# 2361098148/LocoManipulationRL

Hardware: AMD Instinct MI355X
Metric: env-steps/sec (whole node), horizontal-locomotion 4096 envs (higher is better)
Workload: dtype f32

## Files before the change

locomanipulationrl_amd/csrc/lm_dynamics.h:

```cpp
#pragma once
#include "lm_samplers.h"

#if defined(LM_STAMPS) && LM_STAMPS != 2
#define LM_STAMP(k) do { __builtin_amdgcn_sched_barrier(0); unsigned long long t_; \
    asm volatile("s_memtime %0\n\ts_waitcnt lgkmcnt(0)" : "=s"(t_) :: "memory"); __builtin_amdgcn_sched_barrier(0); \
    if (threadIdx.x == 0) { lm_stamp_lds[k] += t_ - lm_stamp_lds[15]; lm_stamp_lds[15] = t_; } } while (0)
#else
#define LM_STAMP(k) do { } while (0)
#endif

#define HUB_FLOATS 10
#define ENVS_PER_WAVE 16
#define PUB_LIMB_STRIDE 123
#define LIMB_STRIDE 124
#define T_J0 0
#define T_P1 14
#define T_P2 40
#define T_I0 66
#define T_Q1 76
#define T_Q2 96
#define T_TIP 116
#define T_FOOT 119
#define T_FLAG 122
#define LM_ITAB_FLOATS (HUB_FLOATS + 4 * LIMB_STRIDE)
// ... 150 lines not shown
  D.H[3] = Hdd.x + 2.0f * g1 * Hdp.x + gg; D.H[4] = -g1 * (Hdp.x + Hdp.y) - gg; D.H[5] = Hdd.y + 2.0f * g1 * Hdp.y + gg;
  const bool on2 = tl[T_FLAG] != 0.f;
  const V3 off = v3(tl[T_FOOT], tl[T_FOOT + 1], tl[T_FOOT + 2]);
  const SV s2 = lo(K.s23), s3 = hi(K.s23), sp1 = lo(K.sp12), sp2_ = hi(K.sp12);
  D.j31 = sel(on2, (-g1) * sp2_, fma6(g1, sp1, s2));
  D.j32 = sel(on2, fma6(g1, sp2_, s3), (-g1) * sp1);
  D.x = sel(on2, hi(K.o32), lo(K.o32)) + mul(M3{sel(on2, hi(K.R32.c0), lo(K.R32.c0)), sel(on2, hi(K.R32.c1), lo(K.R32.c1)), sel(on2, hi(K.R32.c2), lo(K.R32.c2))}, off);
}

struct PgsData { f2 W0t, nrWt; float X0[4][3]; f2 X12[4][3]; };

struct R4 { f2 p, q; };
struct S6 { f2 a, b, c; };
LM_DEV S6 operator*(float s, S6 x) { const f2 t = sp2(s); S6 r; r.a = t * x.a; r.b = t * x.b; r.c = t * x.c; return r; }
LM_DEV S6 fma6(float s, S6 x, S6 y) { const f2 t = sp2(s); S6 r; r.a = fma_(t, x.a, y.a); r.b = fma_(t, x.b, y.b); r.c = fma_(t, x.c, y.c); return r; }
template <int I> LM_DEV float comp(const S6& x) { return I == 0 ? x.a.x : I == 1 ? x.a.y : I == 2 ? x.b.x : I == 3 ? x.b.y : I == 4 ? x.c.x : x.c.y; }
template <int J> LM_DEV f2 pairc(const S6& x) { return J == 0 ? x.a : J == 1 ? x.b : x.c; }

struct Chol6 { float L[6][6]; float d[6]; };
LM_DEV void chol6(const float A[6][6], Chol6& C) {
#pragma unroll
  for (int j = 0; j < 6; j++) {
    float s = A[j][j];
#pragma unroll
    for (int k = 0; k < j; k++) s = fmaf(-C.L[j][k], C.L[j][k], s);
    const float inv = __builtin_amdgcn_rsqf(s);
    C.d[j] = inv;
#pragma unroll
    for (int i = j + 1; i < 6; i++) {
      float t = A[j][i];
#pragma unroll
      for (int k = 0; k < j; k++) t = fmaf(-C.L[i][k], C.L[j][k], t);
      C.L[i][j] = t * inv;
    }
  }
}
LM_DEV void chol6_solve4(const Chol6& C, R4 x[6]) {
#pragma unroll
  for (int i = 0; i < 6; i++) {
    f2 p = x[i].p, q = x[i].q;
#pragma unroll
    for (int k = 0; k < i; k++) { const f2 l = sp2(-C.L[i][k]); p = fma_(l, x[k].p, p); q = fma_(l, x[k].q, q); }
    const f2 d = sp2(C.d[i]); x[i].p = p * d; x[i].q = q * d;
  }
#pragma unroll
  for (int i = 5; i >= 0; i--) {
    f2 p = x[i].p, q = x[i].q;
#pragma unroll
    for (int k = i + 1; k < 6; k++) { const f2 l = sp2(-C.L[k][i]); p = fma_(l, x[k].p, p); q = fma_(l, x[k].q, q); }
    const f2 d = sp2(C.d[i]); x[i].p = p * d; x[i].q = q * d;
  }
}

template <int K>
LM_DEV void pgs_cross_blocks(int limb, const R4 T[6], const R4 X[6], const float Wf[6], float X0[3], f2 X12[3]) {
  float a00 = 0.f; f2 a0t = sp2(0.f), c0 = sp2(0.f), c1 = sp2(0.f), c2 = sp2(0.f);
#pragma unroll
  for (int i = 0; i < 6; i++) {
    const float k0 = quad_bcast<K>(X[i].p.y); const f2 k12 = mk2(quad_bcast<K>(X[i].q.x), quad_bcast<K>(X[i].q.y));
    const float t0 = T[i].p.y; const f2 t12 = T[i].q;
    a00 = fmaf(t0, k0, a00); a0t = fma_(sp2(t0), k12, a0t);
    c0 = fma_(t12, sp2(k0), c0); c1 = fma_(t12, sp2(k12.x), c1); c2 = fma_(t12, sp2(k12.y), c2);
  }
  const bool own = (limb == K);
  X0[0] = own ? Wf[0] : a00; X0[1] = own ? Wf[1] : a0t.x; X0[2] = own ? Wf[2] : a0t.y;
  X12[0] = mk2(own ? Wf[1] : c0.x, own ? Wf[2] : c0.y);
  X12[1] = mk2(own ? Wf[3] : c1.x, own ? Wf[4] : c1.y);
  X12[2] = mk2(own ? Wf[4] : c2.x, own ? Wf[5] : c2.y);
}

template <int K>
LM_DEV void pgs_turn(float m, const PgsData& G, float& lam0, f2& lam12, float& c0, f2& c12) {
  const float d0 = __builtin_amdgcn_fmed3f(c0, -lam0, __builtin_inff());
  lam0 = fmaf(m, d0, lam0);
  const f2 u12 = fma_(fma_(G.W0t, sp2(d0), c12), G.nrWt, lam12);
  const float sc = fminf(1.0f, lam0 * __builtin_amdgcn_rsqf(fmaf(u12.x, u12.x, u12.y * u12.y)));
  const f2 d12 = fma_(u12, sp2(sc), -lam12);
  lam12 = fma_(sp2(m), d12, lam12);
  const float b0 = quad_bcast<K>(d0), b1 = quad_bcast<K>(d12.x), b2 = quad_bcast<K>(d12.y);
  c0 = fmaf(G.X0[K][2], b2, fmaf(G.X0[K][1], b1, fmaf(G.X0[K][0], b0, c0)));
  c12 = fma_(G.X12[K][2], sp2(b2), fma_(G.X12[K][1], sp2(b1), fma_(G.X12[K][0], sp2(b0), c12)));
}

struct PgsState { PgsData G; float lam0; f2 lam12; float c0; f2 c12; float m0, m1, m2, m3; };
LM_DEV void pgs_setup(PgsState& S, int limb, float mu, float bn, const float vf[3], const float Wl[6], const R4 T[6], const R4 X[6]) {
  PgsData& G = S.G; float Wf[6];
  {
    f2 a0 = sp2(0.f), a1 = sp2(0.f), a2 = sp2(0.f); float b0 = 0.f;
#pragma unroll
    for (int i = 0; i < 6; i++) {
      b0 = fmaf(T[i].p.y, X[i].p.y, b0);
      a0 = fma_(sp2(T[i].p.y), X[i].q, a0); a1 = fma_(sp2(T[i].q.x), X[i].q, a1); a2 = fma_(sp2(T[i].q.y), X[i].q, a2);
    }
    Wf[0] = Wl[0] + b0; Wf[1] = Wl[1] + a0.x; Wf[2] = Wl[2] + a0.y;
    Wf[3] = Wl[3] + a1.x; Wf[4] = Wl[4] + a1.y; Wf[5] = Wl[5] + a2.y;
  }
  const float imu = mu > 0.f ? 1.0f / mu : 0.f;
  const float nrW0 = -1.0f / Wf[0]; G.W0t = mk2(Wf[1], Wf[2]); G.nrWt = mk2(-imu / Wf[3], -imu / Wf[5]);
  pgs_cross_blocks<0>(limb, T, X, Wf, G.X0[0], G.X12[0]); pgs_cross_blocks<1>(limb, T, X, Wf, G.X0[1], G.X12[1]);
  pgs_cross_blocks<2>(limb, T, X, Wf, G.X0[2], G.X12[2]); pgs_cross_blocks<3>(limb, T, X, Wf, G.X0[3], G.X12[3]);
#pragma unroll
  for (int k = 0; k < 4; k++) { G.X0[k][0] *= nrW0; G.X0[k][1] *= mu * nrW0; G.X0[k][2] *= mu * nrW0; G.X12[k][1] = sp2(mu) * G.X12[k][1]; G.X12[k][2] = sp2(mu) * G.X12[k][2]; }
  S.lam0 = 0.f; S.lam12 = sp2(0.f);
  S.c0 = (vf[0] + bn) * nrW0; S.c12 = mk2(vf[1], vf[2]);
  S.m0 = limb == 0 ? 1.f : 0.f; S.m1 = limb == 1 ? 1.f : 0.f; S.m2 = limb == 2 ? 1.f : 0.f; S.m3 = limb == 3 ? 1.f : 0.f;
}
LM_DEV void pgs_sweeps(PgsState& S, int it0, int it1) {
  for (int it = it0; it < it1; it += 2) {
    pgs_turn<0>(S.m0, S.G, S.lam0, S.lam12, S.c0, S.c12);
    pgs_turn<1>(S.m1, S.G, S.lam0, S.lam12, S.c0, S.c12);
    pgs_turn<2>(S.m2, S.G, S.lam0, S.lam12, S.c0, S.c12);
    pgs_turn<3>(S.m3, S.G, S.lam0, S.lam12, S.c0, S.c12);
    if (it + 1 < it1) {
      pgs_turn<3>(S.m3, S.G, S.lam0, S.lam12, S.c0, S.c12);
      pgs_turn<2>(S.m2, S.G, S.lam0, S.lam12, S.c0, S.c12);
      pgs_turn<1>(S.m1, S.G, S.lam0, S.lam12, S.c0, S.c12);
      pgs_turn<0>(S.m0, S.G, S.lam0, S.lam12, S.c0, S.c12);
    }
  }
}
LM_DEV void pgs_finish(const PgsState& S, float mu, const R4 X[6], float lam[3], float w[6]) {
  const f2 l12 = sp2(mu) * S.lam12;
  lam[0] = S.lam0; lam[1] = l12.x; lam[2] = l12.y;
#pragma unroll
  for (int i = 0; i < 6; i++) { const f2 t = l12 * X[i].q; w[i] = quad_sum(fmaf(S.lam0, X[i].p.y, t.x + t.y)); }
}

struct FreeBody { V3 p; Q4 q; SV u; };

LM_DEV void integrate_free(FreeBody& F, const M3& R, float dt) {
  V3 ww = mul(R, F.u.w);
  float wn = sqrtf(dot(ww, ww)), th = wn * dt;
  Q4 dq;
  if (th < 1e-8f) { dq.w = 1.f; dq.x = 0.5f * dt * ww.x; dq.y = 0.5f * dt * ww.y; dq.z = 0.5f * dt * ww.z; }
  else { float sh, ch; lm_sincos(0.5f * th, &sh, &ch); float s = sh / wn; dq.w = ch; dq.x = s * ww.x; dq.y = s * ww.y; dq.z = s * ww.z; }
  Q4 qn = qmul(dq, F.q);
  float rn = rsqrtf(qn.w * qn.w + qn.x * qn.x + qn.y * qn.y + qn.z * qn.z);
  F.q.w = qn.w * rn; F.q.x = qn.x * rn; F.q.y = qn.y * rn; F.q.z = qn.z * rn;
  M3 Rn = quat_to_mat(F.q.w, F.q.x, F.q.y, F.q.z);
  F.p = fma3(dt, mul(Rn, F.u.v), F.p);
}

#ifdef LM_WAVES2
#define STASH_SLOTS 18
#define LM_STEP_ATTR __attribute__((amdgpu_waves_per_eu(2, 2)))
#elif defined(LM_HELPER_WAVE)
#if LM_HELPER_WAVE >= 2
#define STASH_SLOTS 34
#define TASK_SLOT 29
#else
#define STASH_SLOTS 29
#endif
#define HAND_IN 22
#define HAND_OUT 26
#define LM_STEP_ATTR
#else
#define STASH_SLOTS 22
#define LM_STEP_ATTR
#endif
struct Stash {
  float4* base; int lane;
  LM_DEV void put(int slot, float a, float b, float c, float d) const { base[slot * 64 + lane] = make_float4(a, b, c, d); }
  LM_DEV float4 get(int slot) const { return base[slot * 64 + lane]; }
};
#ifdef LM_HELPER_WAVE
LM_DEV void hw_barrier() {
  __builtin_amdgcn_sched_barrier(0);
  asm volatile("" ::: "memory");
  __builtin_amdgcn_s_waitcnt(0xc07f);
  __builtin_amdgcn_s_barrier();
  asm volatile("" ::: "memory");
  __builtin_amdgcn_sched_barrier(0);
}
#endif
LM_DEV void stash_sv3(const Stash& S, int slot, SV a, SV b, SV c, float e0 = 0.f, float e1 = 0.f) {
  S.put(slot + 0, a.w.x, a.w.y, a.w.z, a.v.x); S.put(slot + 1, a.v.y, a.v.z, b.w.x, b.w.y);
  S.put(slot + 2, b.w.z, b.v.x, b.v.y, b.v.z); S.put(slot + 3, c.w.x, c.w.y, c.w.z, c.v.x); S.put(slot + 4, c.v.y, c.v.z, e0, e1);
}
LM_DEV void unstash_sv3(const Stash& S, int slot, SV& a, SV& b, SV& c) {
  float4 t0 = S.get(slot), t1 = S.get(slot + 1), t2 = S.get(slot + 2), t3 = S.get(slot + 3), t4 = S.get(slot + 4);
  a = sv(v3(t0.x, t0.y, t0.z), v3(t0.w, t1.x, t1.y)); b = sv(v3(t1.z, t1.w, t2.x), v3(t2.y, t2.z, t2.w)); c = sv(v3(t3.x, t3.y, t3.z), v3(t3.w, t4.x, t4.y));
}

#if defined(LM_PASS0_STASH) || defined(LM_WAVES2)
#define LM_PASS0_REG 0
#else
#define LM_PASS0_REG 1
#endif
struct PassTerms {
  S6 Fq0, Fq1, Fq2;
  float Ha[6], hq[3];
  float Jq0[3]; f2 j12[3];
  R4 PB[6];
  SI Isc;
};
LM_DEV S6 s6(SV a) { S6 r; r.a = mk2(a.w.x, a.w.y); r.b = mk2(a.w.z, a.v.x); r.c = mk2(a.v.y, a.v.z); return r; }
#define LM_PASS_ROWS(I, b, r0, r1, r2) { \
  I.PB[0].p = mk2(b.w.x, r0.w.x); I.PB[1].p = mk2(b.w.y, r0.w.y); I.PB[2].p = mk2(b.w.z, r0.w.z); \
  I.PB[3].p = mk2(b.v.x, r0.v.x); I.PB[4].p = mk2(b.v.y, r0.v.y); I.PB[5].p = mk2(b.v.z, r0.v.z); \
  I.PB[0].q = mk2(r1.w.x, r2.w.x); I.PB[1].q = mk2(r1.w.y, r2.w.y); I.PB[2].q = mk2(r1.w.z, r2.w.z); \
  I.PB[3].q = mk2(r1.v.x, r2.v.x); I.PB[4].q = mk2(r1.v.y, r2.v.y); I.PB[5].q = mk2(r1.v.z, r2.v.z); }
LM_DEV void pin(float& x) { asm("" : "+v"(x)); }
// ... 38 lines not shown
  St.put(4, I.Fq2.c.x, I.Fq2.c.y, 0.f, 0.f);
  St.put(5, I.Ha[0], I.Ha[1], I.Ha[2], I.Ha[3]); St.put(6, I.Ha[4], I.Ha[5], 0.f, 0.f);
  St.put(16, I.Isc.m, I.Isc.h.x, I.Isc.h.y, I.Isc.h.z); St.put(17, I.Isc.xx, I.Isc.yy, I.Isc.zz, I.Isc.xy); St.put(18, I.Isc.xz, I.Isc.yz, 0.f, 0.f);
}
#endif
template <int MODE> LM_DEV void unstash_terms(const Stash& St, PassTerms& I) {
  asm volatile("" ::: "memory");
  float isc_xz = 0.f, isc_yz = 0.f;
  {
    const float4 t0 = St.get(0), t1 = St.get(1), t2 = St.get(2), t3 = St.get(3), t4 = St.get(4);
    isc_xz = t4.z; isc_yz = t4.w;
    I.Fq0.a = mk2(t0.x, t0.y); I.Fq0.b = mk2(t0.z, t0.w); I.Fq0.c = mk2(t1.x, t1.y);
    I.Fq1.a = mk2(t1.z, t1.w); I.Fq1.b = mk2(t2.x, t2.y); I.Fq1.c = mk2(t2.z, t2.w);
    I.Fq2.a = mk2(t3.x, t3.y); I.Fq2.b = mk2(t3.z, t3.w); I.Fq2.c = mk2(t4.x, t4.y);
  }
  const float4 h5 = St.get(5), h6 = St.get(6), h7 = St.get(7), h8 = St.get(8), h9 = St.get(9);
  I.Ha[0] = h5.x; I.Ha[1] = h5.y; I.Ha[2] = h5.z; I.Ha[3] = h5.w; I.Ha[4] = h6.x; I.Ha[5] = h6.y;
  I.hq[0] = h6.z; I.hq[1] = h6.w; I.hq[2] = h7.x;
  I.Jq0[0] = h7.y; I.Jq0[1] = h7.z; I.Jq0[2] = h7.w;
  I.j12[0] = mk2(h8.x, h8.y); I.j12[1] = mk2(h8.z, h8.w); I.j12[2] = mk2(h9.x, h9.y);
  {
    const float4 g0 = St.get(10), g1 = St.get(11), g2 = St.get(12), g3 = St.get(13), g4 = St.get(14), g5 = St.get(15);
    I.PB[0].p = mk2(g0.x, g0.y); I.PB[1].p = mk2(g0.z, g0.w); I.PB[2].p = mk2(g1.x, g1.y); I.PB[3].p = mk2(g1.z, g1.w); I.PB[4].p = mk2(g2.x, g2.y); I.PB[5].p = mk2(g2.z, g2.w);
    I.PB[0].q = mk2(g3.x, g3.y); I.PB[1].q = mk2(g3.z, g3.w); I.PB[2].q = mk2(g4.x, g4.y); I.PB[3].q = mk2(g4.z, g4.w); I.PB[4].q = mk2(g5.x, g5.y); I.PB[5].q = mk2(g5.z, g5.w);
  }
  if (MODE == 0) {
#ifdef LM_WAVES2
    const float4 g16 = St.get(16), g17 = St.get(17), g18 = make_float4(isc_xz, isc_yz, 0.f, 0.f);
#else
    const float4 g16 = St.get(16), g17 = St.get(17), g18 = St.get(18); (void)isc_xz; (void)isc_yz;
#endif
    I.Isc.m = g16.x; I.Isc.h = v3(g16.y, g16.z, g16.w); I.Isc.xx = g17.x; I.Isc.yy = g17.y; I.Isc.zz = g17.z; I.Isc.xy = g17.w; I.Isc.xz = g18.x; I.Isc.yz = g18.y;
  }
}

template <class T> struct PlateInvT { V3T<T> ii, c; T im; };
LM_DEV PlateInvT<float> plate_inv(const lm_params* __restrict__ P, float m, float s) {
  PlateInvT<float> Q; Q.ii = v3(1.0f / (s * P->plate_inertia[0]), 1.0f / (s * P->plate_inertia[1]), 1.0f / (s * P->plate_inertia[2]));
  Q.c = v3(P->plate_com[0], P->plate_com[1], P->plate_com[2]); Q.im = 1.0f / m; return Q;
}
template <class T> LM_DEV void plate_inv_apply(const PlateInvT<T>& Q, V3T<T> n, V3T<T> f, V3T<T>& al, V3T<T>& a) {
  const V3T<T> nc = n - cross(Q.c, f);
  al = v3t<T>(nc.x * Q.ii.x, nc.y * Q.ii.y, nc.z * Q.ii.z);
  a = fma3(Q.im, f, cross(Q.c, al));
}
LM_DEV SI plate_inertia_env(const lm_params* __restrict__ P, float m, float s) {
  const V3 c = v3(P->plate_com[0], P->plate_com[1], P->plate_com[2]); const float cc = dot(c, c);
  SI I; I.m = m; I.h = m * c;
  I.xx = fmaf(m, cc - c.x * c.x, s * P->plate_inertia[0]); I.yy = fmaf(m, cc - c.y * c.y, s * P->plate_inertia[1]); I.zz = fmaf(m, cc - c.z * c.z, s * P->plate_inertia[2]);
  I.xy = -m * c.x * c.y; I.xz = -m * c.x * c.z; I.yz = -m * c.y * c.z;
  return I;
}

template <int MODE, int VAR, int DR, int CF, int HW = 0>
LM_DEV void substep_pass(const lm_params* __restrict__ P, int limb, const FreeBody& F, const PassTerms& I, float dt, float kd, const float cjv[3],
                         const bool sat[3], const float tsat[3], const float tgt[3], const float qd[3], float bn, float mu_dr,
                         bool mp_on, float m_plate, float s_plate, float qdn[3], SV& un, float lamc[3], const Stash* Hd = nullptr) {
  const S6 Fq0 = I.Fq0, Fq1 = I.Fq1, Fq2 = I.Fq2;
  float Ha[6] = {I.Ha[0], I.Ha[1], I.Ha[2], I.Ha[3], I.Ha[4], I.Ha[5]}, r[3];
  const float hq[3] = {I.hq[0], I.hq[1], I.hq[2]};
  R4 PBh[6];
  const float Jq_[3][3] = {{I.Jq0[0], I.Jq0[1], I.Jq0[2]}, {I.j12[0].x, I.j12[1].x, I.j12[2].x}, {I.j12[0].y, I.j12[1].y, I.j12[2].y}};
  const f2 j12_[3] = {I.j12[0], I.j12[1], I.j12[2]};
  float Jqh[3][3]; f2 j12h[3]; float bnh = bn;
  const float (*Jq)[3] = HW == 2 ? Jqh : Jq_;
  const f2* j12 = HW == 2 ? j12h : j12_;
  const R4* PB = HW ? PBh : I.PB;
  const int di[3] = {0, 3, 5};
#pragma unroll
  for (int a = 0; a < 3; a++) {
    const float cj = cjv[a];
    {
#pragma clang fp contract(off)
      Ha[di[a]] = fmaf(dt, sat[a] ? cj : kd + cj, Ha[di[a]]);
      const float rr = sat[a] ? tsat[a] : kd * (tgt[a] - qd[a]);
      const float damp = cj * qd[a];
      r[a] = HW ? rr - damp : (rr - damp) - hq[a];
    }
  }
  float Hi[6]; inv3sym(Ha, Hi);
  const S6 K0 = fma6(Hi[0], Fq0, fma6(Hi[1], Fq1, Hi[2] * Fq2));
  const S6 K1 = fma6(Hi[1], Fq0, fma6(Hi[3], Fq1, Hi[4] * Fq2));
  const S6 K2 = fma6(Hi[2], Fq0, fma6(Hi[4], Fq1, Hi[5] * Fq2));
  float qdd[3], qdf[3], v0f[6], vf[3];
  R4 T[6], X[6];
  if (MODE == 0) {
    float A0[6][6]; si_to_66(I.Isc, A0);
    float A[6][6];
#define LM_AROW(I) { \
      const f2 k0 = sp2(comp<I>(K0)), k1 = sp2(comp<I>(K1)), k2 = sp2(comp<I>(K2)); \
      _Pragma("unroll") for (int jp = (I) / 2; jp < 3; jp++) { \
        const f2 f0 = jp == 0 ? Fq0.a : jp == 1 ? Fq0.b : Fq0.c, f1 = jp == 0 ? Fq1.a : jp == 1 ? Fq1.b : Fq1.c, f2_ = jp == 0 ? Fq2.a : jp == 1 ? Fq2.b : Fq2.c; \
        const f2 v = fma_(-k2, f2_, fma_(-k1, f1, fma_(-k0, f0, mk2(A0[I][2 * jp], A0[I][2 * jp + 1])))); \
        if (2 * jp >= (I)) A[I][2 * jp] = quad_sum(v.x); \
        A[I][2 * jp + 1] = quad_sum(v.y); } }
    LM_AROW(0) LM_AROW(1) LM_AROW(2) LM_AROW(3) LM_AROW(4) LM_AROW(5)
#undef LM_AROW
#ifdef LM_HELPER_WAVE
    if (HW) {
      hw_barrier();
      const float4 b0 = Hd->get(HAND_OUT), b1 = Hd->get(HAND_OUT + 1), b2 = Hd->get(HAND_OUT + 2);
      const float fcs[6] = {b0.x, b0.y, b0.z, b0.w, b1.x, b1.y}, hqh[3] = {b1.z, b1.w, b2.x};
      if (HW == 2) {
        const float4 t7 = Hd->get(7), t8 = Hd->get(8), t9 = Hd->get(9);
        const float4 g0 = Hd->get(10), g1 = Hd->get(11), g2 = Hd->get(12), g3 = Hd->get(13), g4 = Hd->get(14), g5 = Hd->get(15);
        j12h[0] = mk2(t8.x, t8.y); j12h[1] = mk2(t8.z, t8.w); j12h[2] = mk2(t9.x, t9.y); bnh = t9.z;
        Jqh[0][0] = t7.y; Jqh[0][1] = t7.z; Jqh[0][2] = t7.w;
#pragma unroll
        for (int c = 0; c < 3; c++) { Jqh[1][c] = j12h[c].x; Jqh[2][c] = j12h[c].y; }
        PBh[0].p = mk2(fcs[0], g0.y); PBh[1].p = mk2(fcs[1], g0.w); PBh[2].p = mk2(fcs[2], g1.y);
        PBh[3].p = mk2(fcs[3], g1.w); PBh[4].p = mk2(fcs[4], g2.y); PBh[5].p = mk2(fcs[5], g2.w);
        PBh[0].q = mk2(g3.x, g3.y); PBh[1].q = mk2(g3.z, g3.w); PBh[2].q = mk2(g4.x, g4.y);
        PBh[3].q = mk2(g4.z, g4.w); PBh[4].q = mk2(g5.x, g5.y); PBh[5].q = mk2(g5.z, g5.w);
      } else {
#pragma unroll
      for (int i = 0; i < 6; i++) { PBh[i].p = mk2(fcs[i], I.PB[i].p.y); PBh[i].q = I.PB[i].q; }
      }
#pragma unroll
      for (int a = 0; a < 3; a++) {
#pragma clang fp contract(off)
        r[a] = r[a] - hqh[a];
      }
    }
#endif
    Chol6 Ch; chol6(A, Ch);
    const f2 cp[3] = {mk2(r[0], -Jq[0][0]), mk2(r[1], -Jq[0][1]), mk2(r[2], -Jq[0][2])};
#define LM_PROW(I) { \
      const f2 k0 = sp2(comp<I>(K0)), k1 = sp2(comp<I>(K1)), k2 = sp2(comp<I>(K2)); \
      T[I].p = fma_(cp[2], k2, fma_(cp[1], k1, fma_(cp[0], k0, PB[I].p))); \
      T[I].q = fma_(-j12[2], k2, fma_(-j12[1], k1, fma_(-j12[0], k0, PB[I].q))); \
      X[I].p = mk2(-quad_sum(T[I].p.x), T[I].p.y); X[I].q = T[I].q; }
    LM_PROW(0) LM_PROW(1) LM_PROW(2) LM_PROW(3) LM_PROW(4) LM_PROW(5)
#undef LM_PROW
    chol6_solve4(Ch, X);
    float t0 = r[0], t1 = r[1], t2 = r[2];
#define LM_TROW(I) { const float a = X[I].p.x; t0 = fmaf(-comp<I>(Fq0), a, t0); t1 = fmaf(-comp<I>(Fq1), a, t1); t2 = fmaf(-comp<I>(Fq2), a, t2); }
    LM_TROW(0) LM_TROW(1) LM_TROW(2) LM_TROW(3) LM_TROW(4) LM_TROW(5)
#undef LM_TROW
    qdd[0] = Hi[0] * t0 + Hi[1] * t1 + Hi[2] * t2; qdd[1] = Hi[1] * t0 + Hi[3] * t1 + Hi[4] * t2; qdd[2] = Hi[2] * t0 + Hi[4] * t1 + Hi[5] * t2;
    const float u6[6] = {F.u.w.x, F.u.w.y, F.u.w.z, F.u.v.x, F.u.v.y, F.u.v.z};
#pragma unroll
    for (int i = 0; i < 6; i++) v0f[i] = fmaf(dt, X[i].p.x, u6[i]);
  } else {
    qdd[0] = Hi[0] * r[0] + Hi[1] * r[1] + Hi[2] * r[2]; qdd[1] = Hi[1] * r[0] + Hi[3] * r[1] + Hi[4] * r[2]; qdd[2] = Hi[2] * r[0] + Hi[4] * r[1] + Hi[5] * r[2];
#pragma unroll
    for (int i = 0; i < 6; i++) { v0f[i] = PB[i].p.x; T[i] = PB[i]; }
    if (mp_on) {
      const PlateInvT<float> Q1 = plate_inv(P, m_plate, s_plate);
      PlateInvT<f2> Q; Q.ii = bc(Q1.ii); Q.c = bc(Q1.c); Q.im = sp2(Q1.im);
      V3P al, ac;
      plate_inv_apply<f2>(Q, v3(T[0].p, T[1].p, T[2].p), v3(T[3].p, T[4].p, T[5].p), al, ac);
      X[0].p = al.x; X[1].p = al.y; X[2].p = al.z; X[3].p = ac.x; X[4].p = ac.y; X[5].p = ac.z;
      plate_inv_apply<f2>(Q, v3(T[0].q, T[1].q, T[2].q), v3(T[3].q, T[4].q, T[5].q), al, ac);
      X[0].q = al.x; X[1].q = al.y; X[2].q = al.z; X[3].q = ac.x; X[4].q = ac.y; X[5].q = ac.z;
    } else {
#pragma unroll
    for (int i = 0; i < 6; i++) {
      f2 bp = sp2(0.f), bq = sp2(0.f);
#pragma unroll
      for (int j = 0; j < 6; j++) { const f2 ph = sp2(P->plate_phi[6 * i + j]); bp = fma_(ph, T[j].p, bp); bq = fma_(ph, T[j].q, bq); }
      X[i].p = bp; X[i].q = bq;
    }
    }
  }
#pragma unroll
  for (int a = 0; a < 3; a++) qdf[a] = fmaf(dt, qdd[a], qd[a]);
  float Wl[6];
  float JH[3][3];
#pragma unroll
  for (int rr = 0; rr < 3; rr++) {
    JH[rr][0] = Jq[rr][0] * Hi[0] + Jq[rr][1] * Hi[1] + Jq[rr][2] * Hi[2];
    JH[rr][1] = Jq[rr][0] * Hi[1] + Jq[rr][1] * Hi[3] + Jq[rr][2] * Hi[4];
    JH[rr][2] = Jq[rr][0] * Hi[2] + Jq[rr][1] * Hi[4] + Jq[rr][2] * Hi[5];
  }
  Wl[0] = JH[0][0] * Jq[0][0] + JH[0][1] * Jq[0][1] + JH[0][2] * Jq[0][2];
  Wl[1] = JH[0][0] * Jq[1][0] + JH[0][1] * Jq[1][1] + JH[0][2] * Jq[1][2];
  Wl[2] = JH[0][0] * Jq[2][0] + JH[0][1] * Jq[2][1] + JH[0][2] * Jq[2][2];
  Wl[3] = JH[1][0] * Jq[1][0] + JH[1][1] * Jq[1][1] + JH[1][2] * Jq[1][2];
  Wl[4] = JH[1][0] * Jq[2][0] + JH[1][1] * Jq[2][1] + JH[1][2] * Jq[2][2];
  Wl[5] = JH[2][0] * Jq[2][0] + JH[2][1] * Jq[2][1] + JH[2][2] * Jq[2][2];
  {
    float a = 0.f; f2 b = sp2(0.f);
#pragma unroll
    for (int i = 0; i < 6; i++) { a = fmaf(PB[i].p.y, v0f[i], a); b = fma_(PB[i].q, sp2(v0f[i]), b); }
    vf[0] = a + (Jq[0][0] * qdf[0] + Jq[0][1] * qdf[1] + Jq[0][2] * qdf[2]);
    vf[1] = b.x + (Jq[1][0] * qdf[0] + Jq[1][1] * qdf[1] + Jq[1][2] * qdf[2]);
    vf[2] = b.y + (Jq[2][0] * qdf[0] + Jq[2][1] * qdf[1] + Jq[2][2] * qdf[2]);
  }
  float lam[3], w[6];
  LM_STAMP(3);
  PgsState S; pgs_setup(S, limb, DR ? mu_dr : P->mu, HW == 2 ? bnh : bn, vf, Wl, T, X);
  pgs_sweeps(S, 0, P->pgs_iters);
  pgs_finish(S, DR ? mu_dr : P->mu, X, lam, w);
  if (CF) { lamc[0] = lam[0]; lamc[1] = lam[1]; lamc[2] = lam[2]; }
  un = sv(v3(v0f[0] + w[0], v0f[1] + w[1], v0f[2] + w[2]), v3(v0f[3] + w[3], v0f[4] + w[4], v0f[5] + w[5]));
#pragma unroll
  for (int a = 0; a < 3; a++) qdn[a] = qdf[a] + JH[0][a] * lam[0] + JH[1][a] * lam[1] + JH[2][a] * lam[2];
  if (MODE == 0) {
#define LM_WROW(I) { qdn[0] = fmaf(-comp<I>(K0), w[I], qdn[0]); qdn[1] = fmaf(-comp<I>(K1), w[I], qdn[1]); qdn[2] = fmaf(-comp<I>(K2), w[I], qdn[2]); }
    LM_WROW(0) LM_WROW(1) LM_WROW(2) LM_WROW(3) LM_WROW(4) LM_WROW(5)
#undef LM_WROW
  }
  LM_STAMP(4);
}

#ifdef LM_HELPER_WAVE
LM_DEV void helper_wave(const lm_params* __restrict__ P, const float* sTab, float4* sStash, int lane, int nsub) {
  const int limb = lane & 3;
  const float* th = sTab; const float* tl = sTab + HUB_FLOATS + limb * LIMB_STRIDE;
  Stash St; St.base = sStash; St.lane = lane;
  const float gravity = P->gravity;
  for (int s = 0; s < nsub; s++) {
    hw_barrier();
    const float4 h0 = St.get(HAND_IN), h1 = St.get(HAND_IN + 1), h2 = St.get(HAND_IN + 2), h3 = St.get(HAND_IN + 3);
    const float q[3] = {h0.x, h0.y, h0.z}, qd[3] = {h0.w, h1.x, h1.y};
    const SV v0 = sv(v3(h1.z, h1.w, h2.x), v3(h2.y, h2.z, h2.w));
    const SV avp0 = sv(v3(0, 0, 0), gravity * v3(h3.x, h3.y, h3.z));
    LimbKin K; limb_kinematics(tl, q, qd, K);
    LimbDyn D; limb_dynamics<0, 2>(tl, K, qd, v0, avp0, D);
    {
      const float m0 = (limb == 0) ? 1.f : 0.f;
      SI I0 = hub_inertia(th);
      I0.m *= m0; I0.h = m0 * I0.h; I0.xx *= m0; I0.yy *= m0; I0.zz *= m0; I0.xy *= m0; I0.xz *= m0; I0.yz *= m0;
      D.fcs = D.fcs + I0 * avp0 + fcross(v0, I0 * v0);
    }
    St.put(HAND_OUT, D.fcs.w.x, D.fcs.w.y, D.fcs.w.z, D.fcs.v.x); St.put(HAND_OUT + 1, D.fcs.v.y, D.fcs.v.z, D.hq[0], D.hq[1]); St.put(HAND_OUT + 2, D.hq[2], 0.f, 0.f, 0.f);
    hw_barrier();
  }
}
#if LM_HELPER_WAVE >= 2
LM_DEV void helper_wave_terms(const lm_params* __restrict__ P, const float* sTab, float4* sStash, int lane, int nsub) {
  const int limb = lane & 3;
  const float* tl = sTab + HUB_FLOATS + limb * LIMB_STRIDE;
  Stash St; St.base = sStash; St.lane = lane;
  const float dt = P->dt, baumgarte = P->baumgarte, max_depen_vel = P->max_depen_vel;
  for (int s = 0; s < nsub; s++) {
    hw_barrier();
    const float4 h0 = St.get(HAND_IN), h1 = St.get(HAND_IN + 1), h2 = St.get(HAND_IN + 2), h3 = St.get(HAND_IN + 3);
    const float q[3] = {h0.x, h0.y, h0.z}, qd[3] = {h0.w, h1.x, h1.y};
    const SV v0 = sv(v3(h1.z, h1.w, h2.x), v3(h2.y, h2.z, h2.w));
    const SV avp0 = sv(v3(0, 0, 0), v3(0, 0, 0));
    LimbKin K; limb_kinematics(tl, q, qd, K);
    LimbDyn D; limb_dynamics<0, 1>(tl, K, qd, v0, avp0, D);
    V3 C0, C1, C2; float phi;
    C0 = v3(h3.x, h3.y, h3.z);
    C1 = rsqrtf(fmaxf(1.0f - C0.x * C0.x, 1.0e-12f)) * v3(1.0f - C0.x * C0.x, -C0.x * C0.y, -C0.x * C0.z);
    C2 = cross(C0, C1);
    phi = h3.w + dot(C0, D.x) - P->tip_radius;
    D.x = fma3(-P->tip_radius, C0, D.x);
    const float bn = (phi >= 0.f) ? phi / dt : fmaxf(baumgarte * phi / dt, -max_depen_vel);
    V3 e0 = K.s1.v + cross(K.s1.w, D.x);
    V3 e1 = D.j31.v + cross(D.j31.w, D.x);
    V3 e2 = D.j32.v + cross(D.j32.w, D.x);
    St.put(7, 0.f, dot(C0, e0), dot(C0, e1), dot(C0, e2));
    St.put(8, dot(C1, e0), dot(C2, e0), dot(C1, e1), dot(C2, e1)); St.put(9, dot(C1, e2), dot(C2, e2), bn, 0.f);
    const V3 n0 = cross(D.x, C0), n1 = cross(D.x, C1), n2 = cross(D.x, C2);
    St.put(10, 0.f, n0.x, 0.f, n0.y); St.put(11, 0.f, n0.z, 0.f, C0.x); St.put(12, 0.f, C0.y, 0.f, C0.z);
    St.put(13, n1.x, n2.x, n1.y, n2.y); St.put(14, n1.z, n2.z, C1.x, C2.x); St.put(15, C1.y, C2.y, C1.z, C2.z);
    hw_barrier();
  }
}
#endif
#endif

template <int MODE, int VAR, int DR, int CF = 0, int REG0 = 1, int HW = 0>
LM_DEV void substep(const lm_params* __restrict__ P, const float* th, const float* tl, int limb, const Stash& St,
                    FreeBody& F, const M3& Rfix, V3 pfix, float q[3], float qd[3], const float tgt[3], float tau_acc[3], const DrPhys& X, float* cf = nullptr) {
  const float dt = P->dt, kd = DR ? X.kd : P->kd;
  const float cjv[3] = {VAR ? (DR ? X.cj[0] : P->joint_damping) : 0.f, VAR ? (DR ? X.cj[1] : P->joint_damping) : 0.f, VAR ? (DR ? X.cj[2] : P->joint_damping) : 0.f};
  const float tmax[3] = {DR ? X.tmax[0] : P->tau_max, DR ? X.tmax[1] : P->tau_max, DR ? X.tmax[2] : P->tau_max};
  const float mu_dr = DR ? X.mu : 0.f;
  const bool mp_on = DR && MODE == 1 && X.mp_on;
  const float m_plate = mp_on ? X.m_plate : 0.f, s_plate = mp_on ? X.s_plate : 0.f;
  M3 Rf = quat_to_mat(F.q.w, F.q.x, F.q.y, F.q.z);
#ifdef LM_HELPER_WAVE
  static_assert(!HW || (MODE == 0 && !DR && LM_PASS0_REG && REG0), "the helper wavefront serves the un-randomised locomotion sub-step with its first pass on registers");
  if (HW) {
    St.put(HAND_IN, q[0], q[1], q[2], qd[0]); St.put(HAND_IN + 1, qd[1], qd[2], F.u.w.x, F.u.w.y); St.put(HAND_IN + 2, F.u.w.z, F.u.v.x, F.u.v.y, F.u.v.z);
    St.put(HAND_IN + 3, Rf.c0.z, Rf.c1.z, Rf.c2.z, HW == 2 ? F.p.z : 0.f);
    hw_barrier();
  }
#endif
  constexpr bool REG0_ = LM_PASS0_REG ? REG0 != 0 : false;
  const float baumgarte = REG0_ ? P->baumgarte : 0.f, max_depen_vel = REG0_ ? P->max_depen_vel : 0.f;
  float bn; PassTerms I;
  {
    M3 Rb; V3 pb; SV v0;
    if (MODE == 0) { Rb = Rf; pb = F.p; v0 = F.u; } else { Rb = Rfix; pb = pfix; v0 = sv(v3(0, 0, 0), v3(0, 0, 0)); }
    SV avp0 = sv(v3(0, 0, 0), DR ? mulT(Rb, -X.g) : P->gravity * row2(Rb));
    LimbKin K; limb_kinematics(tl, q, qd, K);
    LimbDyn D;
    if (DR && X.mb_on) limb_dynamics<1>(tl, K, qd, v0, avp0, D, X.m_s, X.m_41, X.m_32);
    else if (HW) limb_dynamics<0, 1>(tl, K, qd, v0, avp0, D);
    else limb_dynamics(tl, K, qd, v0, avp0, D);
    LM_STAMP(1);
    if (MODE == 0) {
      const float m0 = (limb == 0) ? 1.f : 0.f;
      SI I0 = hub_inertia(th);
      if (DR && X.mb_on) {
        const V3 c = (1.0f / I0.m) * I0.h; const float dm = X.m_hub - I0.m, cc = dot(c, c);
        I0.xx = fmaf(dm, cc - c.x * c.x, I0.xx); I0.yy = fmaf(dm, cc - c.y * c.y, I0.yy); I0.zz = fmaf(dm, cc - c.z * c.z, I0.zz);
        I0.xy = fmaf(dm, -(c.x * c.y), I0.xy); I0.xz = fmaf(dm, -(c.x * c.z), I0.xz); I0.yz = fmaf(dm, -(c.y * c.z), I0.yz);
        I0.h = (X.m_hub / I0.m) * I0.h; I0.m = X.m_hub;
      }
      const V3 com0 = (1.0f / I0.m) * I0.h;
      I0.m *= m0; I0.h = m0 * I0.h; I0.xx *= m0; I0.yy *= m0; I0.zz *= m0; I0.xy *= m0; I0.xz *= m0; I0.yz *= m0;
      D.Isc = D.Isc + I0;
      if (!HW) D.fcs = D.fcs + I0 * avp0 + fcross(v0, I0 * v0);
      if (DR) { V3 fh = m0 * mulT(Rb, X.f); D.fcs = D.fcs - sv(cross(com0, fh), fh); }
    }
#ifdef LM_HELPER_WAVE
    if (HW == 2) {
// ... 192 lines not shown
```

locomanipulationrl_amd/csrc/lm_engine_h3.hip:

```cpp
#ifndef LM_HELPER_WAVE
#define LM_HELPER_WAVE 2
#endif
#ifndef LM_H3_OUT_HELPER
#define LM_H3_OUT_HELPER 1
#endif
#ifndef LM_H3_TAIL_STATE
#define LM_H3_TAIL_STATE 1
#endif
#undef LM_STAMPS
#undef LM_COUNT_PASS2
#undef LM_WAVES2
#undef LM_PASS0_STASH
#include "lm_step.h"

__global__ void __launch_bounds__(192) k_step_h3(StepArgs A) {
  LM_STEP_SMEM(64)
  if (threadIdx.x >= 64) {
    const int nsub = (A.nsub < 0) ? P->substeps : A.nsub;
    if (kind != 0 || env0 >= A.N) return;
    if (threadIdx.x >= 128) {
      helper_wave_terms(P, sTab, sStash, threadIdx.x - 128, nsub);
      if (LM_H3_TAIL_STATE) hw_barrier();
      if (LM_H3_OUT_HELPER) helper_write_outputs<64>(P, A.W, A.N, env0, threadIdx.x - 128, sObs, sSt);
    } else {
      helper_wave(P, sTab, sStash, threadIdx.x - 64, nsub);
      if (LM_H3_TAIL_STATE) helper_task_state(A, P, sStash, threadIdx.x - 64);
    }
    return;
  }
  if (kind == 0) step_body<0, 0, 0, 0, 0, 1, 2, LM_H3_OUT_HELPER, 0, LM_H3_TAIL_STATE>(A, P, sTab, sObs, sSt, sStash); else step_body<1, 0, 0>(A, P, sTab, sObs, sSt, sStash);
}
extern "C" __attribute__((visibility("hidden"))) void lm_internal_launch_step_h3(const StepArgs* A, int nblocks, hipStream_t s) {
  hipLaunchKernelGGL(k_step_h3, dim3(nblocks), dim3(192), 0, s, *A);
}
```

Baseline: 149.9 million.

## Offload PGS cross-limb coupling blocks to helper wavefronts in the h3 kernel

The main wavefront now does the 6x6 Cholesky factorisation first and writes it, together with its K rows, into the LDS stash. The two helper wavefronts each rebuild T and X, do the Cholesky solve and compute the raw cross-limb coupling blocks for two of the four limbs. The main wave then fetches these blocks after a barrier and only applies the per-limb selection and scaling, which takes the per-limb cross-block FMA chains off its critical path. In exchange the stash grows from 34 to 49 slots, there are extra helper barriers every substep, and the solve is repeated on the helper waves. The feature is enabled by default in the h3 engine.

Result: faster. 152.9 million, median of 6 (+2.0%).

```diff
diff --git a/locomanipulationrl_amd/csrc/lm_dynamics.h b/locomanipulationrl_amd/csrc/lm_dynamics.h
--- a/locomanipulationrl_amd/csrc/lm_dynamics.h
+++ b/locomanipulationrl_amd/csrc/lm_dynamics.h
@@ -226,8 +226,9 @@
   }
 }
 
+struct XRaw { float a00; f2 a0t, c0, c1, c2; };
 template <int K>
-LM_DEV void pgs_cross_blocks(int limb, const R4 T[6], const R4 X[6], const float Wf[6], float X0[3], f2 X12[3]) {
+LM_DEV void pgs_cross_raw(const R4 T[6], const R4 X[6], XRaw& R) {
   float a00 = 0.f; f2 a0t = sp2(0.f), c0 = sp2(0.f), c1 = sp2(0.f), c2 = sp2(0.f);
 #pragma unroll
   for (int i = 0; i < 6; i++) {
@@ -236,11 +237,19 @@
     a00 = fmaf(t0, k0, a00); a0t = fma_(sp2(t0), k12, a0t);
     c0 = fma_(t12, sp2(k0), c0); c1 = fma_(t12, sp2(k12.x), c1); c2 = fma_(t12, sp2(k12.y), c2);
   }
+  R.a00 = a00; R.a0t = a0t; R.c0 = c0; R.c1 = c1; R.c2 = c2;
+}
+template <int K>
+LM_DEV void pgs_cross_select(int limb, const XRaw& R, const float Wf[6], float X0[3], f2 X12[3]) {
   const bool own = (limb == K);
-  X0[0] = own ? Wf[0] : a00; X0[1] = own ? Wf[1] : a0t.x; X0[2] = own ? Wf[2] : a0t.y;
-  X12[0] = mk2(own ? Wf[1] : c0.x, own ? Wf[2] : c0.y);
-  X12[1] = mk2(own ? Wf[3] : c1.x, own ? Wf[4] : c1.y);
-  X12[2] = mk2(own ? Wf[4] : c2.x, own ? Wf[5] : c2.y);
+  X0[0] = own ? Wf[0] : R.a00; X0[1] = own ? Wf[1] : R.a0t.x; X0[2] = own ? Wf[2] : R.a0t.y;
+  X12[0] = mk2(own ? Wf[1] : R.c0.x, own ? Wf[2] : R.c0.y);
+  X12[1] = mk2(own ? Wf[3] : R.c1.x, own ? Wf[4] : R.c1.y);
+  X12[2] = mk2(own ? Wf[4] : R.c2.x, own ? Wf[5] : R.c2.y);
+}
+template <int K>
+LM_DEV void pgs_cross_blocks(int limb, const R4 T[6], const R4 X[6], const float Wf[6], float X0[3], f2 X12[3]) {
+  XRaw R; pgs_cross_raw<K>(T, X, R); pgs_cross_select<K>(limb, R, Wf, X0, X12);
 }
 
 template <int K>
@@ -257,7 +266,17 @@
 }
 
 struct PgsState { PgsData G; float lam0; f2 lam12; float c0; f2 c12; float m0, m1, m2, m3; };
-LM_DEV void pgs_setup(PgsState& S, int limb, float mu, float bn, const float vf[3], const float Wl[6], const R4 T[6], const R4 X[6]) {
+#ifndef LM_H3_XBLOCKS
+#define LM_H3_XBLOCKS 0
+#endif
+struct Stash;
+#if defined(LM_HELPER_WAVE) && LM_HELPER_WAVE >= 2
+LM_DEV void xblocks_fetch(const Stash* Hd, XRaw& R0, XRaw& R1, XRaw& R2, XRaw& R3);
+#endif
+LM_DEV void pin_here(float& x) { asm volatile("" : "+v"(x)); }
+LM_DEV void pin_here(f2& x) { asm volatile("" : "+v"(x)); }
+template <int XB = 0>
+LM_DEV void pgs_setup(PgsState& S, int limb, float mu, float bn, const float vf[3], const float Wl[6], const R4 T[6], const R4 X[6], const Stash* Hd = nullptr) {
   PgsData& G = S.G; float Wf[6];
   {
     f2 a0 = sp2(0.f), a1 = sp2(0.f), a2 = sp2(0.f); float b0 = 0.f;
@@ -270,13 +289,25 @@
     Wf[3] = Wl[3] + a1.x; Wf[4] = Wl[4] + a1.y; Wf[5] = Wl[5] + a2.y;
   }
   const float imu = mu > 0.f ? 1.0f / mu : 0.f;
-  const float nrW0 = -1.0f / Wf[0]; G.W0t = mk2(Wf[1], Wf[2]); G.nrWt = mk2(-imu / Wf[3], -imu / Wf[5]);
+  float nrW0 = -1.0f / Wf[0]; G.W0t = mk2(Wf[1], Wf[2]); G.nrWt = mk2(-imu / Wf[3], -imu / Wf[5]);
+#if defined(LM_HELPER_WAVE) && LM_HELPER_WAVE >= 2
+  if (XB) {
+    S.c0 = (vf[0] + bn) * nrW0; S.c12 = mk2(vf[1], vf[2]);
+    pin_here(Wf[0]); pin_here(Wf[1]); pin_here(Wf[2]); pin_here(Wf[3]); pin_here(Wf[4]); pin_here(Wf[5]);
+    pin_here(nrW0); pin_here(G.nrWt); pin_here(S.c0); pin_here(S.c12);
+    XRaw R0, R1, R2, R3; xblocks_fetch(Hd, R0, R1, R2, R3);
+    pgs_cross_select<0>(limb, R0, Wf, G.X0[0], G.X12[0]); pgs_cross_select<1>(limb, R1, Wf, G.X0[1], G.X12[1]);
+    pgs_cross_select<2>(limb, R2, Wf, G.X0[2], G.X12[2]); pgs_cross_select<3>(limb, R3, Wf, G.X0[3], G.X12[3]);
+  } else
+#endif
+  {
   pgs_cross_blocks<0>(limb, T, X, Wf, G.X0[0], G.X12[0]); pgs_cross_blocks<1>(limb, T, X, Wf, G.X0[1], G.X12[1]);
   pgs_cross_blocks<2>(limb, T, X, Wf, G.X0[2], G.X12[2]); pgs_cross_blocks<3>(limb, T, X, Wf, G.X0[3], G.X12[3]);
+  }
 #pragma unroll
   for (int k = 0; k < 4; k++) { G.X0[k][0] *= nrW0; G.X0[k][1] *= mu * nrW0; G.X0[k][2] *= mu * nrW0; G.X12[k][1] = sp2(mu) * G.X12[k][1]; G.X12[k][2] = sp2(mu) * G.X12[k][2]; }
   S.lam0 = 0.f; S.lam12 = sp2(0.f);
-  S.c0 = (vf[0] + bn) * nrW0; S.c12 = mk2(vf[1], vf[2]);
+  if (!XB) { S.c0 = (vf[0] + bn) * nrW0; S.c12 = mk2(vf[1], vf[2]); }
   S.m0 = limb == 0 ? 1.f : 0.f; S.m1 = limb == 1 ? 1.f : 0.f; S.m2 = limb == 2 ? 1.f : 0.f; S.m3 = limb == 3 ? 1.f : 0.f;
 }
 LM_DEV void pgs_sweeps(PgsState& S, int it0, int it1) {
@@ -320,8 +351,15 @@
 #define LM_STEP_ATTR __attribute__((amdgpu_waves_per_eu(2, 2)))
 #elif defined(LM_HELPER_WAVE)
 #if LM_HELPER_WAVE >= 2
+#define TASK_SLOT 29
+#if LM_H3_XBLOCKS
+#define STASH_SLOTS 49
+#define XB_IN_A TASK_SLOT
+#define XB_IN_B 34
+#define XB_OUT 39
+#else
 #define STASH_SLOTS 34
-#define TASK_SLOT 29
+#endif
 #else
 #define STASH_SLOTS 29
 #endif
@@ -466,6 +504,11 @@
   return I;
 }
 
+#define LM_PROW(I, BIAS) { \
+      const f2 k0 = sp2(comp<I>(K0)), k1 = sp2(comp<I>(K1)), k2 = sp2(comp<I>(K2)); \
+      T[I].p = fma_(cp[2], k2, fma_(cp[1], k1, fma_(cp[0], k0, PB[I].p))); \
+      T[I].q = fma_(-j12[2], k2, fma_(-j12[1], k1, fma_(-j12[0], k0, PB[I].q))); \
+      X[I].p = mk2(BIAS, T[I].p.y); X[I].q = T[I].q; }
 template <int MODE, int VAR, int DR, int CF, int HW = 0>
 LM_DEV void substep_pass(const lm_params* __restrict__ P, int limb, const FreeBody& F, const PassTerms& I, float dt, float kd, const float cjv[3],
                          const bool sat[3], const float tsat[3], const float tgt[3], const float qd[3], float bn, float mu_dr,
@@ -510,8 +553,18 @@
         A[I][2 * jp + 1] = quad_sum(v.y); } }
     LM_AROW(0) LM_AROW(1) LM_AROW(2) LM_AROW(3) LM_AROW(4) LM_AROW(5)
 #undef LM_AROW
+    Chol6 Ch;
 #ifdef LM_HELPER_WAVE
     if (HW) {
+#if LM_HELPER_WAVE >= 2 && LM_H3_XBLOCKS
+      if (HW == 2) {
+        chol6(A, Ch);
+        put2(*Hd, XB_IN_A, K0.a, K0.b); put2(*Hd, XB_IN_A + 1, K0.c, K1.a); put2(*Hd, XB_IN_A + 2, K1.b, K1.c); put2(*Hd, XB_IN_A + 3, K2.a, K2.b);
+        Hd->put(XB_IN_A + 4, K2.c.x, K2.c.y, Ch.d[0], Ch.d[1]); Hd->put(XB_IN_B, Ch.d[2], Ch.d[3], Ch.d[4], Ch.d[5]);
+        Hd->put(XB_IN_B + 1, Ch.L[1][0], Ch.L[2][0], Ch.L[2][1], Ch.L[3][0]); Hd->put(XB_IN_B + 2, Ch.L[3][1], Ch.L[3][2], Ch.L[4][0], Ch.L[4][1]);
+        Hd->put(XB_IN_B + 3, Ch.L[4][2], Ch.L[4][3], Ch.L[5][0], Ch.L[5][1]); Hd->put(XB_IN_B + 4, Ch.L[5][2], Ch.L[5][3], Ch.L[5][4], 0.f);
+      }
+#endif
       hw_barrier();
       const float4 b0 = Hd->get(HAND_OUT), b1 = Hd->get(HAND_OUT + 1), b2 = Hd->get(HAND_OUT + 2);
       const float fcs[6] = {b0.x, b0.y, b0.z, b0.w, b1.x, b1.y}, hqh[3] = {b1.z, b1.w, b2.x};
@@ -537,15 +590,10 @@
       }
     }
 #endif
-    Chol6 Ch; chol6(A, Ch);
+    if (!(HW == 2 && LM_H3_XBLOCKS)) chol6(A, Ch);
     const f2 cp[3] = {mk2(r[0], -Jq[0][0]), mk2(r[1], -Jq[0][1]), mk2(r[2], -Jq[0][2])};
-#define LM_PROW(I) { \
-      const f2 k0 = sp2(comp<I>(K0)), k1 = sp2(comp<I>(K1)), k2 = sp2(comp<I>(K2)); \
-      T[I].p = fma_(cp[2], k2, fma_(cp[1], k1, fma_(cp[0], k0, PB[I].p))); \
-      T[I].q = fma_(-j12[2], k2, fma_(-j12[1], k1, fma_(-j12[0], k0, PB[I].q))); \
-      X[I].p = mk2(-quad_sum(T[I].p.x), T[I].p.y); X[I].q = T[I].q; }
-    LM_PROW(0) LM_PROW(1) LM_PROW(2) LM_PROW(3) LM_PROW(4) LM_PROW(5)
-#undef LM_PROW
+    LM_PROW(0, -quad_sum(T[0].p.x)) LM_PROW(1, -quad_sum(T[1].p.x)) LM_PROW(2, -quad_sum(T[2].p.x))
+    LM_PROW(3, -quad_sum(T[3].p.x)) LM_PROW(4, -quad_sum(T[4].p.x)) LM_PROW(5, -quad_sum(T[5].p.x))
     chol6_solve4(Ch, X);
     float t0 = r[0], t1 = r[1], t2 = r[2];
 #define LM_TROW(I) { const float a = X[I].p.x; t0 = fmaf(-comp<I>(Fq0), a, t0); t1 = fmaf(-comp<I>(Fq1), a, t1); t2 = fmaf(-comp<I>(Fq2), a, t2); }
@@ -603,8 +651,10 @@
   }
   float lam[3], w[6];
   LM_STAMP(3);
-  PgsState S; pgs_setup(S, limb, DR ? mu_dr : P->mu, HW == 2 ? bnh : bn, vf, Wl, T, X);
-  pgs_sweeps(S, 0, P->pgs_iters);
+  constexpr int XB = (HW == 2 && LM_H3_XBLOCKS) ? 1 : 0;
+  const int iters = XB ? P->pgs_iters : 0;
+  PgsState S; pgs_setup<XB>(S, limb, DR ? mu_dr : P->mu, HW == 2 ? bnh : bn, vf, Wl, T, X, Hd);
+  pgs_sweeps(S, 0, XB ? iters : P->pgs_iters);
   pgs_finish(S, DR ? mu_dr : P->mu, X, lam, w);
   if (CF) { lamc[0] = lam[0]; lamc[1] = lam[1]; lamc[2] = lam[2]; }
   un = sv(v3(v0f[0] + w[0], v0f[1] + w[1], v0f[2] + w[2]), v3(v0f[3] + w[3], v0f[4] + w[4], v0f[5] + w[5]));
@@ -619,6 +669,45 @@
 }
 
 #ifdef LM_HELPER_WAVE
+#if LM_HELPER_WAVE >= 2
+LM_DEV void xblocks_fetch(const Stash* Hd, XRaw& R0, XRaw& R1, XRaw& R2, XRaw& R3) {
+#if LM_H3_XBLOCKS
+  hw_barrier();
+  const float4 a0 = Hd->get(XB_OUT), a1 = Hd->get(XB_OUT + 1), a2 = Hd->get(XB_OUT + 2), a3 = Hd->get(XB_OUT + 3), a4 = Hd->get(XB_OUT + 4);
+  const float4 b0 = Hd->get(XB_OUT + 5), b1 = Hd->get(XB_OUT + 6), b2 = Hd->get(XB_OUT + 7), b3 = Hd->get(XB_OUT + 8), b4 = Hd->get(XB_OUT + 9);
+  R0.a00 = a0.x; R0.a0t = mk2(a0.y, a0.z); R0.c0 = mk2(a0.w, a1.x); R0.c1 = mk2(a1.y, a1.z); R0.c2 = mk2(a1.w, a2.x);
+  R1.a00 = a2.y; R1.a0t = mk2(a2.z, a2.w); R1.c0 = mk2(a3.x, a3.y); R1.c1 = mk2(a3.z, a3.w); R1.c2 = mk2(a4.x, a4.y);
+  R2.a00 = b0.x; R2.a0t = mk2(b0.y, b0.z); R2.c0 = mk2(b0.w, b1.x); R2.c1 = mk2(b1.y, b1.z); R2.c2 = mk2(b1.w, b2.x);
+  R3.a00 = b2.y; R3.a0t = mk2(b2.z, b2.w); R3.c0 = mk2(b3.x, b3.y); R3.c1 = mk2(b3.z, b3.w); R3.c2 = mk2(b4.x, b4.y);
+#endif
+}
+#if LM_H3_XBLOCKS
+template <int KA, int KB>
+LM_DEV void helper_xblocks(const Stash& St, int out) {
+  const float4 i0 = St.get(XB_IN_A), i1 = St.get(XB_IN_A + 1), i2 = St.get(XB_IN_A + 2), i3 = St.get(XB_IN_A + 3), i4 = St.get(XB_IN_A + 4);
+  const float4 i5 = St.get(XB_IN_B), i6 = St.get(XB_IN_B + 1), i7 = St.get(XB_IN_B + 2), i8 = St.get(XB_IN_B + 3), i9 = St.get(XB_IN_B + 4);
+  const float4 t7 = St.get(7), t8 = St.get(8), t9 = St.get(9);
+  const float4 g0 = St.get(10), g1 = St.get(11), g2 = St.get(12), g3 = St.get(13), g4 = St.get(14), g5 = St.get(15);
+  S6 K0, K1, K2;
+  K0.a = mk2(i0.x, i0.y); K0.b = mk2(i0.z, i0.w); K0.c = mk2(i1.x, i1.y); K1.a = mk2(i1.z, i1.w); K1.b = mk2(i2.x, i2.y); K1.c = mk2(i2.z, i2.w);
+  K2.a = mk2(i3.x, i3.y); K2.b = mk2(i3.z, i3.w); K2.c = mk2(i4.x, i4.y);
+  Chol6 Ch;
+  Ch.d[0] = i4.z; Ch.d[1] = i4.w; Ch.d[2] = i5.x; Ch.d[3] = i5.y; Ch.d[4] = i5.z; Ch.d[5] = i5.w;
+  Ch.L[1][0] = i6.x; Ch.L[2][0] = i6.y; Ch.L[2][1] = i6.z; Ch.L[3][0] = i6.w; Ch.L[3][1] = i7.x; Ch.L[3][2] = i7.y; Ch.L[4][0] = i7.z; Ch.L[4][1] = i7.w;
+  Ch.L[4][2] = i8.x; Ch.L[4][3] = i8.y; Ch.L[5][0] = i8.z; Ch.L[5][1] = i8.w; Ch.L[5][2] = i9.x; Ch.L[5][3] = i9.y; Ch.L[5][4] = i9.z;
+  const f2 cp[3] = {mk2(0.f, -t7.y), mk2(0.f, -t7.z), mk2(0.f, -t7.w)};
+  const f2 j12[3] = {mk2(t8.x, t8.y), mk2(t8.z, t8.w), mk2(t9.x, t9.y)};
+  R4 PB[6], T[6], X[6];
+  PB[0].p = mk2(0.f, g0.y); PB[1].p = mk2(0.f, g0.w); PB[2].p = mk2(0.f, g1.y); PB[3].p = mk2(0.f, g1.w); PB[4].p = mk2(0.f, g2.y); PB[5].p = mk2(0.f, g2.w);
+  PB[0].q = mk2(g3.x, g3.y); PB[1].q = mk2(g3.z, g3.w); PB[2].q = mk2(g4.x, g4.y); PB[3].q = mk2(g4.z, g4.w); PB[4].q = mk2(g5.x, g5.y); PB[5].q = mk2(g5.z, g5.w);
+  LM_PROW(0, 0.f) LM_PROW(1, 0.f) LM_PROW(2, 0.f) LM_PROW(3, 0.f) LM_PROW(4, 0.f) LM_PROW(5, 0.f)
+  chol6_solve4(Ch, X);
+  XRaw A, B; pgs_cross_raw<KA>(T, X, A); pgs_cross_raw<KB>(T, X, B);
+  St.put(out, A.a00, A.a0t.x, A.a0t.y, A.c0.x); St.put(out + 1, A.c0.y, A.c1.x, A.c1.y, A.c2.x); St.put(out + 2, A.c2.y, B.a00, B.a0t.x, B.a0t.y);
+  St.put(out + 3, B.c0.x, B.c0.y, B.c1.x, B.c1.y); St.put(out + 4, B.c2.x, B.c2.y, 0.f, 0.f);
+}
+#endif
+#endif
 LM_DEV void helper_wave(const lm_params* __restrict__ P, const float* sTab, float4* sStash, int lane, int nsub) {
   const int limb = lane & 3;
   const float* th = sTab; const float* tl = sTab + HUB_FLOATS + limb * LIMB_STRIDE;
@@ -640,6 +729,10 @@
     }
     St.put(HAND_OUT, D.fcs.w.x, D.fcs.w.y, D.fcs.w.z, D.fcs.v.x); St.put(HAND_OUT + 1, D.fcs.v.y, D.fcs.v.z, D.hq[0], D.hq[1]); St.put(HAND_OUT + 2, D.hq[2], 0.f, 0.f, 0.f);
     hw_barrier();
+#if LM_HELPER_WAVE >= 2 && LM_H3_XBLOCKS
+    helper_xblocks<2, 3>(St, XB_OUT + 5);
+    hw_barrier();
+#endif
   }
 }
 #if LM_HELPER_WAVE >= 2
@@ -672,6 +765,10 @@
     St.put(10, 0.f, n0.x, 0.f, n0.y); St.put(11, 0.f, n0.z, 0.f, C0.x); St.put(12, 0.f, C0.y, 0.f, C0.z);
     St.put(13, n1.x, n2.x, n1.y, n2.y); St.put(14, n1.z, n2.z, C1.x, C2.x); St.put(15, C1.y, C2.y, C1.z, C2.z);
     hw_barrier();
+#if LM_H3_XBLOCKS
+    helper_xblocks<0, 1>(St, XB_OUT);
+    hw_barrier();
+#endif
   }
 }
 #endif
diff --git a/locomanipulationrl_amd/csrc/lm_engine_h3.hip b/locomanipulationrl_amd/csrc/lm_engine_h3.hip
--- a/locomanipulationrl_amd/csrc/lm_engine_h3.hip
+++ b/locomanipulationrl_amd/csrc/lm_engine_h3.hip
@@ -1,5 +1,8 @@
 #ifndef LM_HELPER_WAVE
 #define LM_HELPER_WAVE 2
+#endif
+#ifndef LM_H3_XBLOCKS
+#define LM_H3_XBLOCKS 1
 #endif
 #ifndef LM_H3_OUT_HELPER
 #define LM_H3_OUT_HELPER 1
```
